# SinOncology/BreakID

Hardware: AMD Instinct MI355X
Metric: M reads/s clustered+split-scanned (higher is better)
Workload: dtype int32/u8 (+f64 sd replay)

## Files before the change

### breakid_amd/capi.py

```python
from __future__ import annotations

import ctypes as C
import math
import os
import subprocess

import numpy as np

from . import abi

_HERE = os.path.dirname(os.path.abspath(__file__))
LIB_PATH = os.path.join(_HERE, "libbreakid_hip.so")
_LIB = None


class BreakIDError(RuntimeError):
    def __init__(self, code, msg):
        super().__init__("libbreakid_hip error %d: %s" % (code, msg))
        self.code = code


def build(verbose=False):
    cmd = ["make", "-C", os.path.join(_HERE, "csrc"), "-j8"]
    r = subprocess.run(cmd, capture_output=not verbose, text=True)
    if r.returncode != 0:
        raise RuntimeError("building libbreakid_hip.so failed:\n" + (r.stdout or "")[-4000:] + (r.stderr or "")[-4000:])


EXPORTS = ["bk_init", "bk_prepare_process", "bk_free", "bk_last_error", "bk_set_stream", "bk_sync", "bk_get_stream", "bk_upload_records", "bk_records", "bk_exclude_regions", "bk_isize_stats",
           "bk_discordant_pairs", "bk_mask_and_cluster", "bk_split_evidence", "bk_cluster_summary",
           "bk_split_breakpoints", "bk_normal_support", "bk_ref_support", "bk_genotype_call", "bk_clip_support", "bk_clip_reads", "bk_base_depth", "bk_clip_rescue", "bk_junctions", "bk_junction_sides", "bk_vcf_breakend_alt", "bk_evidence", "bk_unique_support", "bk_clip_consensus", "bk_junction_fit", "bk_locus_similarity", "bk_site_complexity", "bk_window_coverage", "bk_window_context", "bk_call_windows", "bk_fusion_frame", "bk_link_calls", "bk_locus_partners", "bk_call_partner_sites", "bk_fragment_sizes", "bk_fragment_bounds", "bk_known_calls", "bk_split_junctions", "bk_split_junction_counts", "bk_debug_split_junctions", "bk_cigar_gaps", "bk_cigar_gap_counts", "bk_run", "bk_fetch", "bk_timing", "bk_timing_enable", "bk_timing_touched", "bk_group_stats", "bk_qname_hash", "bk_qname_check",
           "bk_bam_open", "bk_bam_header", "bk_bam_decode", "bk_bam_close", "bk_bam_extract", "bk_bam_names_free", "bk_bam_reads", "bk_reads_free", "bk_bam_decode_device", "bk_bam_decode_device_part", "bk_bam_decode_device_ctx", "bk_bam_dev_free", "bk_feed_release_caches", "bk_debug_bgzf_inflate", "bk_debug_std_sort", "bk_debug_scan", "bk_debug_radix_sort", "bk_debug_prims_info", "bk_sort_forms", "bk_debug_ahc", "bk_debug_points", "bk_debug_points_groups", "bk_debug_cluster_info", "bk_debug_stream_info", "bk_debug_stream_blocks", "bk_debug_cigar", "bk_debug_vote", "bk_debug_region", "bk_shard_begin", "bk_shard_get_stats", "bk_shard_set_stats",
           "bk_shard_sd_local", "bk_shard_sd_finish", "bk_shard_buffer", "bk_shard_set_buffer", "bk_shard_group_sizes",
           "bk_shard_own_groups", "bk_shard_route_candidates", "bk_shard_group_keys", "bk_shard_route_pairs", "bk_shard_group_pairs", "bk_shard_bp_cov", "bk_shard_bp_vote", "bk_shard_bp_vote_slice", "bk_shard_bp_set_voted", "bk_shard_bp_depth", "bk_shard_bp_finish"]


def lib():
    global _LIB
    if _LIB is None:
        if not os.path.exists(LIB_PATH):
            raise BreakIDError(abi.BK_ERR_NO_DEVICE, "libbreakid_hip.so is not built (run __graft_entry__.build()); "
                                                     "there is no CPU fallback")
        try:
            import torch
        except Exception:
            pass
        L = C.CDLL(LIB_PATH)
        vp, u64p, dp = C.c_void_p, C.POINTER(C.c_uint64), C.POINTER(C.c_double)
        L.bk_init.argtypes = [C.c_int, vp, C.POINTER(C.c_char_p), C.c_int, C.POINTER(vp)]
        L.bk_free.argtypes = [vp]
        L.bk_last_error.restype = C.c_char_p
        L.bk_last_error.argtypes = [vp]
        L.bk_set_stream.argtypes = [vp, vp]
        L.bk_sync.argtypes = [vp]
        L.bk_upload_records.argtypes = [vp, C.POINTER(abi.Soa), C.c_int]
# ... 26 lines not shown
        L.bk_window_context.argtypes = [vp, vp, C.c_uint64, C.c_int, C.POINTER(vp)]
        L.bk_call_windows.argtypes = [vp, C.c_int, C.c_int, C.c_uint32, vp, vp]
        L.bk_fusion_frame.argtypes = [vp, C.POINTER(abi.TxModel), vp, C.c_uint64, C.POINTER(vp)]
        L.bk_link_calls.argtypes = [vp, vp, C.c_uint64, C.c_uint32, C.POINTER(vp)]
        L.bk_locus_partners.argtypes = [vp, vp, C.c_uint64, C.c_uint32, C.POINTER(vp)]
        L.bk_call_partner_sites.argtypes = [vp, C.c_double, vp]
        L.bk_fragment_sizes.argtypes = [vp, vp, C.c_uint64, C.c_int32, C.c_int32, C.POINTER(vp)]
        L.bk_fragment_bounds.argtypes = [C.c_double, C.c_double, C.POINTER(C.c_int32), C.POINTER(C.c_int32)]
        L.bk_known_calls.argtypes = [vp, vp, C.c_uint64, vp, C.c_uint64, C.c_uint32, C.POINTER(vp)]
        L.bk_split_junctions.argtypes = [vp, C.c_int, C.c_uint32, C.c_uint32, C.POINTER(vp), u64p]
        L.bk_split_junction_counts.argtypes = [vp, u64p]
        L.bk_debug_split_junctions.argtypes = [vp, C.c_int, C.c_uint32, C.c_uint32, vp, C.c_uint64, C.POINTER(vp), u64p]
        L.bk_cigar_gaps.argtypes = [vp, C.c_int, C.c_uint32, C.c_uint32, C.c_uint32, C.c_uint32, C.POINTER(vp), u64p]
        L.bk_cigar_gap_counts.argtypes = [vp, u64p]
        L.bk_fetch.argtypes = [vp, C.c_int, C.POINTER(vp), u64p, C.POINTER(C.POINTER(C.c_uint64)), C.POINTER(C.c_uint32)]
        L.bk_timing.argtypes = [vp, C.POINTER(C.POINTER(C.c_char_p)), C.POINTER(C.POINTER(C.c_float)),
                                C.POINTER(C.POINTER(C.c_uint64)), C.POINTER(C.c_int)]
        L.bk_timing_enable.argtypes = [vp, C.c_int]
        L.bk_timing_touched.argtypes = [vp, C.POINTER(C.POINTER(C.c_uint64)), C.POINTER(C.c_int)]
        L.bk_debug_std_sort.argtypes = [vp, vp, vp, C.c_uint32, vp]
        L.bk_debug_scan.argtypes = [vp, C.c_int, vp, C.c_uint64, C.c_int, vp]
        L.bk_debug_radix_sort.argtypes = [vp, vp, vp, C.c_uint64, C.c_int, C.c_int, vp, vp]
        L.bk_debug_prims_info.argtypes = [u64p]
        L.bk_sort_forms.argtypes = [vp, u64p]
        L.bk_debug_ahc.argtypes = [vp, vp, vp, C.c_uint32, C.c_double, vp, vp, C.POINTER(C.c_uint32)]
        L.bk_debug_points.argtypes = [vp, C.c_int, vp, vp, C.c_uint32, C.c_double, vp, vp, C.POINTER(C.c_uint32)]
        L.bk_debug_points_groups.argtypes = [vp, C.c_int, vp, vp, vp, C.c_uint32, C.c_double, vp, vp, vp, C.POINTER(C.c_uint32)]
        L.bk_debug_cluster_info.argtypes = [u64p]
        L.bk_debug_stream_info.argtypes = [u64p]
        L.bk_debug_stream_blocks.argtypes = [C.c_uint]
        L.bk_debug_cigar.argtypes = [vp, C.c_uint32, vp, vp, vp, vp, vp, vp, vp]
        L.bk_debug_vote.argtypes = [vp, vp, C.c_uint32, vp, C.c_uint32, C.c_int32, C.c_int32, vp]
        L.bk_debug_region.argtypes = [vp, C.c_int32, C.c_uint32, C.c_uint32, C.c_uint64, vp, C.c_uint32, C.POINTER(C.c_uint32), C.POINTER(C.c_uint32),
                                      C.POINTER(C.c_uint32)]
        L.bk_shard_begin.argtypes = [vp, C.c_uint64, C.c_int]
        L.bk_shard_get_stats.argtypes = [vp, C.POINTER(abi.ShardStats)]
        L.bk_shard_set_stats.argtypes = [vp, C.POINTER(abi.ShardStats)]
        L.bk_shard_sd_local.argtypes = [vp, u64p, C.POINTER(vp), u64p]
        L.bk_shard_sd_finish.argtypes = [vp, vp, C.c_uint64, C.c_uint64, dp, dp]
        L.bk_shard_buffer.argtypes = [vp, C.c_int, C.POINTER(vp), u64p, C.POINTER(C.c_uint32)]
        L.bk_shard_set_buffer.argtypes = [vp, C.c_int, vp, C.c_uint64]
        L.bk_shard_group_sizes.argtypes = [vp, C.POINTER(C.POINTER(C.c_uint64)), C.POINTER(C.c_uint32)]
        L.bk_shard_own_groups.argtypes = [vp, vp, C.c_uint32]
        L.bk_shard_route_candidates.argtypes = [vp, C.c_uint32, C.POINTER(vp), C.POINTER(C.POINTER(C.c_uint64))]
        L.bk_shard_group_keys.argtypes = [vp, C.POINTER(C.POINTER(C.c_uint32)), C.POINTER(C.c_uint32)]
        L.bk_shard_route_pairs.argtypes = [vp, vp, C.c_uint32, C.c_uint32, C.POINTER(vp), C.POINTER(C.POINTER(C.c_uint64))]
# ... 71 lines not shown
    rc = M.bk_multi_run(C.byref(soa), lens.ctypes.data, names, len(contigs), int(n_gpus), int(transport), int(qual), int(fast), C.byref(w), C.byref(ncl), C.byref(h), err, 512)
    if rc != 0:
        raise BreakIDError(rc, err.value.decode())
    try:
        mean, sd = C.c_double(), C.c_double()
        rc = M.bk_multi_stats(h, C.byref(mean), C.byref(sd), None, None)
        if rc != 0:
            raise BreakIDError(rc, "bk_multi_stats")
        L = lib()
        clusters, _ = abi.fetch_array(L, h, lambda hh, st, d, c, g, ng: L.bk_fetch(hh, st, d, c, g, ng), abi.STAGE_CLUSTERS)
        return {"w": w.value, "n_clustered": ncl.value, "mean": mean.value, "sd": sd.value, "clusters": clusters}
    finally:
        M.bk_multi_free(h)


def prims_info():
    out = (C.c_uint64 * 4)()
    rc = lib().bk_debug_prims_info(out)
    if rc != 0:
        raise BreakIDError(rc, "bk_debug_prims_info")
    return dict(zip(("BLOCK", "SCAN_TILE", "SCAN_ONE_MAX", "RS_TILE"), (int(v) for v in out)))


def cluster_info():
    out = (C.c_uint64 * 2)()
    rc = lib().bk_debug_cluster_info(out)
    if rc != 0:
        raise BreakIDError(rc, "bk_debug_cluster_info")
    return dict(zip(("FW_TILE", "FW_LEVELS"), (int(v) for v in out)))


def stream_info():
    out = (C.c_uint64 * 4)()
    rc = lib().bk_debug_stream_info(out)
    if rc != 0:
        raise BreakIDError(rc, "bk_debug_stream_info")
    return dict(zip(("STREAM_V", "ST_CAND_CAP", "ST_SA_CAP", "RESIDENT"), (int(v) for v in out)))


def stream_blocks(blocks):
    rc = lib().bk_debug_stream_blocks(int(blocks))
    if rc != 0:
        raise BreakIDError(rc, "bk_debug_stream_blocks")


def w_from(mean, sd):
# ... 471 lines not shown

    def debug_std_sort(self, key, group_off):
        key = np.ascontiguousarray(key, np.uint32)
        group_off = np.ascontiguousarray(group_off, np.uint64)
        perm = np.zeros(len(key), np.uint32)
        self._check(self.L.bk_debug_std_sort(self.h, key.ctypes.data, group_off.ctypes.data, len(group_off) - 1, perm.ctypes.data))
        return perm

    def debug_scan(self, values, in_place=False):
        values = np.ascontiguousarray(values)
        assert values.ndim == 1 and values.dtype in (np.uint32, np.uint64), values.dtype
        out = np.zeros(len(values) + 1, values.dtype)
        self._check(self.L.bk_debug_scan(self.h, values.dtype.itemsize, values.ctypes.data if len(values) else None, len(values), int(in_place), out.ctypes.data))
        return out

    def debug_radix_sort(self, keys, vals, begin_bit, end_bit):
        keys = np.ascontiguousarray(keys, np.uint64)
        vals = np.ascontiguousarray(vals, np.uint32)
        assert keys.ndim == 1 and keys.shape == vals.shape
        n = len(keys)
        ko, vo = np.zeros(n, np.uint64), np.zeros(n, np.uint32)
        self._check(self.L.bk_debug_radix_sort(self.h, keys.ctypes.data if n else None, vals.ctypes.data if n else None, n, int(begin_bit), int(end_bit),
                                               ko.ctypes.data if n else None, vo.ctypes.data if n else None))
        return ko, vo

    def sort_forms(self):
        out = (C.c_uint64 * 3)()
        self._check(self.L.bk_sort_forms(self.h, out))
        return tuple(int(v) for v in out)

    def debug_ahc(self, x, y, w):
        x = np.ascontiguousarray(x, np.uint32)
        y = np.ascontiguousarray(y, np.uint32)
        n = len(x)
        idx = np.zeros(max(n, 1), np.uint32)
        cl = np.zeros(max(n, 1), np.int32)
        m = C.c_uint32()
        self._check(self.L.bk_debug_ahc(self.h, x.ctypes.data, y.ctypes.data, n, float(w), idx.ctypes.data, cl.ctypes.data, C.byref(m)))
        return idx[:m.value].copy(), cl[:m.value].copy()

    def debug_points(self, mode, x, y, w):
        x = np.ascontiguousarray(x, np.uint32)
        y = np.ascontiguousarray(y, np.uint32)
        n = len(x)
        idx = np.zeros(max(n, 1), np.uint32)
        cl = np.zeros(max(n, 1), np.int32)
# ... 308 lines not shown
```

### breakid_amd/csrc/api.hip

```cpp
#include <algorithm>
#include <cmath>
#include <limits>
#include <cstring>
#include <numeric>

#include "bk_common.h"
#include "prims.h"
#include "stream.h"
#include "join.h"
#include "cluster.h"
#include "bp.h"
#include "normal.h"
#include "genotype.h"
#include "clip.h"
#include "junction.h"
#include "evidence.h"
#include "unique.h"
#include "consensus.h"
#include "jfit.h"
#include "locsim.h"
#include "seqcx.h"
#include "coverage.h"
#include "context.h"
#include "frame.h"
// ... 130 lines not shown
  std::vector<struct bk_window_cov> f_wincov;
  CtxBufs cxb;
  std::vector<struct bk_window_ctx> f_winctx;
  FrameBufs frb;
  std::vector<struct bk_frame_call> f_frame;
  LinkBufs lkb;
  std::vector<struct bk_call_link> f_link;
  PartnerBufs ptb;
  std::vector<struct bk_locus_partners> f_partners;
  FragBufs fgb;
  std::vector<struct bk_frag_sizes> f_fragsize;
  KnownBufs knb;
  std::vector<struct bk_known_call> f_known;
  SjBufs sjb;
  SjStats sj_stats;
  std::vector<SjClaim> sj_claims;
  bool sj_claims_valid = false;
  std::vector<struct bk_split_junction> f_sj;
  GapBufs gpb;
  GapStats gap_stats;
  std::vector<struct bk_cigar_gap> f_gaps;

  prims::RadixBufs dbg_radix;
  DevBuf dbg_in, dbg_out, dbg_vals;

  std::vector<bk_pair> f_pairs[3];
  std::vector<uint64_t> f_off[3];
  std::vector<bk_split> f_splits;
  std::vector<bk_cluster> f_clusters;
  std::vector<int32_t> f_gkeys;
  std::vector<bk_group_stat> f_gstats;

  bool timing = false;
  std::vector<StageTimer> timers;
  Timing tout;

  void tick(const char *name, uint64_t bytes, bool begin, uint64_t touched = 0)
  {
    if (!timing) return;
    if (begin)
    {
      StageTimer t;
      t.name = name;
      t.bytes = bytes;
      t.touched = touched;
      HIP_CHECK(hipEventCreate(&t.a));
// ... 2203 lines not shown
    prims::RadixBufs &rb = ctx->dbg_radix;
    uint64_t *dk = ctx->dbg_in.as<uint64_t>(n);
    uint32_t *dv = ctx->dbg_vals.as<uint32_t>(n);
    HIP_CHECK(hipMemsetAsync(rb.keys_alt.as<uint64_t>(n), 0xA5, n * 8, ctx->st));
    HIP_CHECK(hipMemsetAsync(rb.vals_alt.as<uint32_t>(n), 0xA5, n * 4, ctx->st));
    HIP_CHECK(hipMemcpyAsync(dk, keys, n * 8, hipMemcpyHostToDevice, ctx->st));
    HIP_CHECK(hipMemcpyAsync(dv, vals, n * 4, hipMemcpyHostToDevice, ctx->st));
    uint64_t *ko = nullptr;
    uint32_t *vo = nullptr;
    prims::radix_sort_pairs(dk, dv, n, begin_bit, end_bit, rb, ctx->st, &ko, &vo);
    HIP_CHECK(hipMemcpyAsync(keys_out, ko, n * 8, hipMemcpyDeviceToHost, ctx->st));
    HIP_CHECK(hipMemcpyAsync(vals_out, vo, n * 4, hipMemcpyDeviceToHost, ctx->st));
    HIP_CHECK(hipStreamSynchronize(ctx->st));
  });
}

int bk_debug_prims_info(uint64_t out[4])
{
  if (!out) return BK_ERR_ARG;
  out[0] = prims::BLOCK;
  out[1] = prims::SCAN_TILE;
  out[2] = prims::SCAN_ONE_MAX;
  out[3] = prims::RS_TILE;
  return BK_OK;
}

int bk_sort_forms(bk_ctx *ctx, uint64_t out[3])
{
  return guarded(ctx, [&] {
    if (!out) throw bk_error(BK_ERR_ARG, "bk_sort_forms: null output");
    ctx->stage.sort_forms(out);
  });
}

int bk_debug_ahc(bk_ctx *ctx, const uint32_t *x, const uint32_t *y, uint32_t n, double w, uint32_t *idx_out, int32_t *cluster_out, uint32_t *n_out)
{
  return guarded(ctx, [&] {
    if (!x || !y || !idx_out || !cluster_out || !n_out) throw bk_error(BK_ERR_ARG, "bk_debug_ahc: null argument");
    std::vector<bk_pair> hp(n);
    for (uint32_t i = 0; i < n; ++i)
    {
      memset(&hp[i], 0, sizeof(bk_pair));
      hp[i].x = x[i];
      hp[i].y = y[i];
    }
    DevBuf dp, dcl;
// ... 436 lines not shown
```

### breakid_amd/csrc/bp.h

```cpp
#pragma once
#include "bk_common.h"
#include "prims.h"

template <class Less> __device__ __forceinline__ uint64_t wave_lower(uint64_t lo, uint64_t hi, Less less)
{
  const uint32_t lane = threadIdx.x & 63;
  while (hi - lo > 64)
  {
    const uint64_t width = hi - lo;
    const uint64_t p = lo + width * (lane + 1) / 65;
    const uint32_t c = (uint32_t) __popcll(__ballot(less(p)));
    const uint64_t nlo = c ? lo + width * c / 65 + 1 : lo;
    const uint64_t nhi = c < 64 ? lo + width * (c + 1) / 65 : hi;
    lo = nlo;
    hi = nhi;
  }
  const uint64_t i = lo + lane;
  return lo + (uint64_t) __popcll(__ballot(i < hi && less(i)));
}
__device__ __forceinline__ uint32_t wave_sum_u32(uint32_t v)
{
  for (int d = 32; d; d >>= 1) v += (uint32_t) __shfl_xor((int) v, d, 64);
  return v;
}

// ... 26 lines not shown
  {
    const unsigned long long want = rec_key(T, P < -0x80000000ll ? -0x80000000ll : P);
    const unsigned long long *__restrict__ samp = r.samp;
    const uint64_t a = wave_lower(0, r.n_samp, [&](uint64_t m) { return samp[m] < want; });
    lo = a ? ((a - 1) << REC_SAMPLE_SHIFT) + 1 : 0;
    hi = a < r.n_samp ? (a << REC_SAMPLE_SHIFT) : r.n;
  }
  const uint32_t Tu = (uint32_t) T;
  return wave_lower(lo, hi, [&](uint64_t m) {
    const uint32_t t = (uint32_t) r.tid[m];
    return t != Tu ? (t < Tu) : ((long long) r.pos[m] < P);
  });
}

struct BpWork
{
  uint64_t t1lo, t1hi, t2lo, t2hi;
  uint32_t ok, pad;
};

struct BpBufs
{
  DevBuf samp, key, val, kmax, lexbase, slotbase, an, as1, as2, amin1, amax1, amin2, amax2, atype, keep, off, tmpc, work, nmatch, moff, err, emit, ecount, scan_tmp, cov, depth, voted, nvalid, maxrec;
  prims::RadixBufs radix;
};

uint64_t count_valid_clusters(const bk_cluster *cl, uint64_t ncl, BpBufs &b, hipStream_t st);
void sort_splits(bk_split *unsorted, uint64_t n, bk_split *sorted, BpBufs &b, hipStream_t st, int rec_bits);
uint64_t cluster_summary(const bk_pair *pairs, const uint32_t *idx, const uint32_t *gof, const uint32_t *cl, uint64_t n, uint32_t ng, const uint32_t *gkey,
                         const uint32_t *glex, const uint32_t *lex_to_num, int32_t nt, double w, DevBuf &clusters_out, BpBufs &b, hipStream_t st);
RecView rec_sampled(const RecView &r, DevBuf &samp, hipStream_t st);
uint32_t *bp_cov_partial(const RecView &r, const bk_cluster *cl, uint64_t ncl, double w, int maxspan, BpBufs &b, hipStream_t st);
void bp_vote(const bk_split *sp, uint64_t nsp, bk_cluster *cl, uint64_t ncl, double w, int maxspan, const uint32_t *cov, const int32_t *hdr_id, BpBufs &b, hipStream_t st);
uint32_t *bp_depth_partial(const RecView &r, const bk_cluster *cl, uint64_t ncl, int maxspan, BpBufs &b, hipStream_t st);
void base_depth_at(const RecView &r, const int32_t *tid, const uint32_t *pos, uint64_t n, int maxspan, DevBuf &samp, hipStream_t st, uint32_t *depth);
void bp_finish(bk_cluster *cl, uint64_t ncl, const uint32_t *depth, BpBufs &b, hipStream_t st);
void split_breakpoints(const RecView &r, const bk_split *sp, uint64_t nsp, bk_cluster *cl, uint64_t ncl, double w, int maxspan, const int32_t *hdr_id, BpBufs &b,
                       hipStream_t st);
void debug_region(const RecView &r, const bk_split *sp, uint64_t nsp, int32_t tid, uint32_t start, uint32_t end, int maxspan, unsigned long long depth_pos, bk_split *out,
                  uint32_t cap, uint32_t *res, hipStream_t st);
```

### breakid_amd/csrc/bp.hip

```cpp
#include "bk_common.h"
#include "prims.h"
#include "bp.h"
#include <algorithm>
#include <vector>

namespace
{
__global__ __launch_bounds__(256) void k_group_kmax(const uint32_t *__restrict__ gof, const uint32_t *__restrict__ cl, uint64_t n, uint32_t *__restrict__ kmax)
{
  uint64_t p = (uint64_t) blockIdx.x * blockDim.x + threadIdx.x;
  const bool live = p < n;
  uint32_t g = live ? gof[p] : 0xFFFFFFFFu;
  uint32_t v = live ? cl[p] + 1 : 0u;
  __shared__ uint32_t s_g[4], s_v[4];
  const uint32_t g0 = __shfl(g, 0, 64);
  const bool wave_uniform = __ballot(live && g != g0) == 0ull;
  if (wave_uniform)
    for (int d = 32; d; d >>= 1) v = max(v, (uint32_t) __shfl_xor((int) v, d, 64));
  if ((threadIdx.x & 63) == 0)
  {
    s_g[threadIdx.x >> 6] = wave_uniform ? g0 : 0xFFFFFFFEu;
    s_v[threadIdx.x >> 6] = v;
  }
  __syncthreads();
// ... 586 lines not shown

void sort_splits(bk_split *unsorted, uint64_t n, bk_split *sorted, BpBufs &b, hipStream_t st, int rec_bits)
{
  if (n == 0) return;
  uint64_t *key = b.key.as<uint64_t>(n);
  uint32_t *val = b.val.as<uint32_t>(n);
  unsigned long long *mx = nullptr;
  if (rec_bits <= 0)
  {
    mx = b.maxrec.as<unsigned long long>(2);
    HIP_CHECK(hipMemsetAsync(mx, 0, 8, st));
  }
  hipLaunchKernelGGL(k_split_keys, dim3(nb(n)), dim3(256), 0, st, unsorted, n, key, val, mx);
  if (mx)
  {
    unsigned long long h = 0;
    HIP_CHECK(hipMemcpyAsync(&h, mx, 8, hipMemcpyDeviceToHost, st));
    HIP_CHECK(hipStreamSynchronize(st));
    rec_bits = 1;
    while (rec_bits < 64 && (h >> rec_bits) != 0ull) ++rec_bits;
  }
  uint64_t *ks;
  uint32_t *vs;
  prims::radix_sort_pairs(key, val, n, 0, rec_bits, b.radix, st, &ks, &vs);
  hipLaunchKernelGGL(k_split_gather, dim3(nb(n)), dim3(256), 0, st, unsorted, vs, n, sorted);
}

uint64_t cluster_summary(const bk_pair *pairs, const uint32_t *idx, const uint32_t *gof, const uint32_t *cl, uint64_t n, uint32_t ng, const uint32_t *gkey,
                         const uint32_t *glex, const uint32_t *lex_to_num, int32_t nt, double w, DevBuf &clusters_out, BpBufs &b, hipStream_t st)
{
  if (n == 0 || ng == 0) return 0;
  uint32_t *kmax = b.kmax.as<uint32_t>((uint64_t) ng + 1);
  HIP_CHECK(hipMemsetAsync(kmax, 0, ((uint64_t) ng + 1) * 4, st));
  hipLaunchKernelGGL(k_group_kmax, dim3(nb(n)), dim3(256), 0, st, gof, cl, n, kmax);
  uint32_t *slotbase = b.slotbase.as<uint32_t>((uint64_t) ng + 1), *lexbase = b.lexbase.as<uint32_t>((uint64_t) ng + 1);
  hipLaunchKernelGGL(k_slot_bases, dim3(1), dim3(prims::BLOCK), 0, st, kmax, lex_to_num, ng, lexbase, slotbase);
  uint32_t nslots = 0;
  HIP_CHECK(hipMemcpyAsync(&nslots, lexbase + ng, 4, hipMemcpyDeviceToHost, st));
  HIP_CHECK(hipStreamSynchronize(st));
  if (nslots == 0) return 0;
  ClusterAcc acc;
  acc.n = b.an.as<uint32_t>(nslots);
  acc.sum1 = b.as1.as<unsigned long long>(nslots);
  acc.sum2 = b.as2.as<unsigned long long>(nslots);
  acc.min1 = b.amin1.as<uint32_t>(nslots);
  acc.max1 = b.amax1.as<uint32_t>(nslots);
  acc.min2 = b.amin2.as<uint32_t>(nslots);
// ... 147 lines not shown
```

### breakid_amd/csrc/join.h

```cpp
#pragma once
#include "bk_common.h"
#include "prims.h"
#include <vector>

struct JoinBufs
{
  DevBuf counter, unsorted, okey, oval, key, val, pairs, gof, gflag, gscan, gstart, gkey, scan_tmp, route_cand, route_cnt, route_pairs, route_off, maxrec, key2, val2;
  prims::RadixBufs radix;
  int rec_bits = 32;
  int rec_bits_eff = 32;
};

struct JoinResult
{
  uint64_t n_pairs = 0;
  uint32_t n_groups = 0;
  bk_pair *pairs = nullptr;
  uint32_t *gof = nullptr;
  uint64_t *gstart = nullptr;
  uint32_t *gkey = nullptr;
};

void join_candidates(const Cand *cand, uint64_t n_cand, double w, const uint32_t *tprefix, int32_t nt, JoinBufs &b, hipStream_t st, JoinResult &res);
void join_assign_ids(JoinResult &res, const uint32_t *glex_dev, hipStream_t st);

Cand *route_candidates(const Cand *cand, uint64_t n, uint32_t world, JoinBufs &b, hipStream_t st, std::vector<uint64_t> &counts);
bk_pair *route_pairs(const JoinResult &jr, const std::vector<uint64_t> &off_of_group, JoinBufs &b, hipStream_t st);
void group_pairs(const bk_pair *raw, uint64_t np, int32_t nt, JoinBufs &b, hipStream_t st, JoinResult &res);
```

### breakid_amd/csrc/join.hip

```cpp
#include "bk_common.h"
#include "prims.h"
#include "join.h"

namespace
{
__global__ __launch_bounds__(256) void k_join_keys(const Cand *__restrict__ c, uint64_t n, uint64_t *__restrict__ key, uint32_t *__restrict__ val)
{
  uint64_t i = (uint64_t) blockIdx.x * blockDim.x + threadIdx.x;
  if (i < n)
  {
    key[i] = c[i].qhash;
    val[i] = (uint32_t) i;
  }
}

__global__ __launch_bounds__(256) void k_join_rec_keys(const Cand *__restrict__ c, uint64_t n, uint64_t *__restrict__ key, uint32_t *__restrict__ val)
{
  uint64_t i = (uint64_t) blockIdx.x * blockDim.x + threadIdx.x;
  if (i < n)
  {
    key[i] = c[i].rec;
    val[i] = (uint32_t) i;
  }
}
// ... 310 lines not shown
{
  if (n_cand > 0xFFFFFFF0ull) throw bk_error(BK_ERR_LIMIT, "more than 2^32 discordant candidates");
  const int rec_bits = effective_rec_bits(cand, n_cand, k_max_rec_cand, nt, b, st);
  unsigned long long *counter = b.counter.as<unsigned long long>(2);
  uint32_t *err = (uint32_t *) (counter + 1);
  HIP_CHECK(hipMemsetAsync(counter, 0, 16, st));
  uint64_t cap = n_cand / 2 + 1;
  bk_pair *unsorted = b.unsorted.as<bk_pair>(cap);
  uint64_t *okey = b.okey.as<uint64_t>(cap);
  uint32_t *oval = b.oval.as<uint32_t>(cap);
  unsigned long long host[2] = {0, 0};
  static const int first_attempt = getenv("BK_JOIN_ATTEMPT") ? std::max(0, std::min(2, atoi(getenv("BK_JOIN_ATTEMPT")))) : 0;
  for (int attempt = first_attempt; attempt < 3; ++attempt)
  {
    if (n_cand)
    {
      uint64_t *key = b.key.as<uint64_t>(n_cand);
      uint32_t *val = b.val.as<uint32_t>(n_cand);
      uint64_t *ks;
      uint32_t *vs;
      if (attempt < 2)
      {
        hipLaunchKernelGGL(k_join_keys, dim3(cdiv(n_cand, 256)), dim3(256), 0, st, cand, n_cand, key, val);
        prims::radix_sort_pairs(key, val, n_cand, attempt == 0 ? 32 : 0, 64, b.radix, st, &ks, &vs);
        if (attempt == 0) hipLaunchKernelGGL(k_join_fix_runs, dim3(cdiv(n_cand, 256)), dim3(256), 0, st, ks, vs, n_cand, err);
      }
      else
      {
        hipLaunchKernelGGL(k_join_rec_keys, dim3(cdiv(n_cand, 256)), dim3(256), 0, st, cand, n_cand, key, val);
        prims::radix_sort_pairs(key, val, n_cand, 0, rec_bits, b.radix, st, &ks, &vs);
        uint64_t *key2 = b.key2.as<uint64_t>(n_cand);
        uint32_t *val2 = b.val2.as<uint32_t>(n_cand);
        hipLaunchKernelGGL(k_join_hash_of, dim3(cdiv(n_cand, 256)), dim3(256), 0, st, cand, (const uint32_t *) vs, n_cand, key2, val2);
        prims::radix_sort_pairs(key2, val2, n_cand, 0, 64, b.radix, st, &ks, &vs);
      }
      hipLaunchKernelGGL(k_join_pairs, dim3(cdiv(n_cand, 256)), dim3(256), 0, st, cand, ks, vs, n_cand, w, tprefix, nt, unsorted, okey, oval,
                         (unsigned long long) cap, counter, err, rec_bits, attempt == 2 ? 1 : 0);
    }
    HIP_CHECK(hipMemcpyAsync(host, counter, 16, hipMemcpyDeviceToHost, st));
    HIP_CHECK(hipStreamSynchronize(st));
    if (attempt == 0 && ((uint32_t) host[1] & 4u))
    {
      HIP_CHECK(hipMemsetAsync(counter, 0, 16, st));
      continue;
    }
    if (attempt < 2 && ((uint32_t) host[1] & 1u) && !((uint32_t) host[1] & 2u))
    {
      HIP_CHECK(hipMemsetAsync(counter, 0, 16, st));
      attempt = 1;
      continue;
    }
    break;
  }
  if ((uint32_t) host[1] & 2u)
    throw bk_error(BK_ERR_COLLISION, "two different read names share one 64-bit name hash (their second hashes differ): the mate join would not be the reference's");
  if ((uint32_t) host[1] & 1u) throw bk_error(BK_ERR_HIP, "mate join: a run was refused although its candidates were sorted (internal error)");
  if (host[0] > cap) throw bk_error(BK_ERR_LIMIT, "pair capacity exceeded");
  return host[0];
}

static void group_sorted(const bk_pair *unsorted, uint64_t *okey, uint32_t *oval, uint64_t np, int32_t nt, JoinBufs &b, hipStream_t st, JoinResult &res)
{
  res = JoinResult();
  res.n_pairs = np;
  bk_pair *pairs = b.pairs.as<bk_pair>(np + 1);
  uint32_t *gof = b.gof.as<uint32_t>(np + 1);
  res.pairs = pairs;
  res.gof = gof;
  if (np == 0) return;
  int gbits = 1;
  while ((1ull << gbits) < (uint64_t) (nt + 1) * (uint64_t) (nt + 1) && gbits < 32) ++gbits;
  uint64_t *ks;
  uint32_t *vs;
  const int rbits = b.rec_bits_eff;
  prims::radix_sort_pairs(okey, oval, np, 0, rbits + gbits, b.radix, st, &ks, &vs);
  uint32_t *gflag = b.gflag.as<uint32_t>(np + 1);
  uint32_t *gscan = b.gscan.as<uint32_t>(np + 1);
  hipLaunchKernelGGL(k_gather_pairs, dim3(cdiv(np, 256)), dim3(256), 0, st, unsorted, vs, ks, np, pairs, gflag, rbits);
  prims::exclusive_scan<uint32_t>(gflag, gscan, np, b.scan_tmp, st);
  uint32_t ng = 0;
  HIP_CHECK(hipMemcpyAsync(&ng, gscan + np, 4, hipMemcpyDeviceToHost, st));
  HIP_CHECK(hipStreamSynchronize(st));
  res.n_groups = ng;
  uint64_t *gstart = b.gstart.as<uint64_t>((uint64_t) ng + 1);
  uint32_t *gkey = b.gkey.as<uint32_t>((uint64_t) ng + 1);
  hipLaunchKernelGGL(k_group_starts, dim3(cdiv(np, 256)), dim3(256), 0, st, gflag, gscan, ks, np, gstart, gkey, gof, rbits);
  res.gstart = gstart;
  res.gkey = gkey;
}

void join_candidates(const Cand *cand, uint64_t n_cand, double w, const uint32_t *tprefix, int32_t nt, JoinBufs &b, hipStream_t st, JoinResult &res)
{
  const uint64_t np = join_raw_pairs(cand, n_cand, w, tprefix, nt, b, st);
  group_sorted(b.unsorted.get<bk_pair>(), b.okey.get<uint64_t>(), b.oval.get<uint32_t>(), np, nt, b, st, res);
}

void group_pairs(const bk_pair *raw, uint64_t np, int32_t nt, JoinBufs &b, hipStream_t st, JoinResult &res)
{
// ... 52 lines not shown
```

### include/breakid_hip.h

```cpp
#ifndef BREAKID_HIP_H
#define BREAKID_HIP_H

#include <stdint.h>
#include <stddef.h>

#ifdef __cplusplus
extern "C" {
#endif

#define BK_OK 0
#define BK_ERR_ARG (-1)
#define BK_ERR_HIP (-2)
#define BK_ERR_NO_DEVICE (-3)
#define BK_ERR_UNSORTED (-4)
#define BK_ERR_CIGAR (-5)
#define BK_ERR_IO (-6)
#define BK_ERR_LIMIT (-7)
#define BK_ERR_COLLISION (-8)

#define BK_MEM_HOST 0
#define BK_MEM_DEVICE 1

typedef struct bk_ctx bk_ctx;

// ... 314 lines not shown
int bk_shard_sd_local(bk_ctx *ctx, uint64_t *l_total, void **ex_dev, uint64_t *n_ex);
int bk_shard_sd_finish(bk_ctx *ctx, const void *all_ex_dev, uint64_t n_all, uint64_t l_grand, double *mean, double *sd);
int bk_shard_buffer(bk_ctx *ctx, int which, void **dev, uint64_t *count, uint32_t *elem_bytes);
int bk_shard_set_buffer(bk_ctx *ctx, int which, const void *dev, uint64_t count);
int bk_shard_group_sizes(bk_ctx *ctx, const uint64_t **starts, uint32_t *n_groups);
int bk_shard_own_groups(bk_ctx *ctx, const uint8_t *own, uint32_t n_groups);
int bk_shard_route_candidates(bk_ctx *ctx, uint32_t world, void **dev, const uint64_t **counts);
int bk_shard_group_keys(bk_ctx *ctx, const uint32_t **keys, uint32_t *n_groups);
int bk_shard_route_pairs(bk_ctx *ctx, const uint32_t *dest_of_group, uint32_t n_groups, uint32_t world, void **dev, const uint64_t **counts);
int bk_shard_group_pairs(bk_ctx *ctx, const void *pairs_dev, uint64_t n, const uint32_t *all_keys, uint32_t n_all_keys);
int bk_shard_bp_cov(bk_ctx *ctx, double w, void **cov_dev, uint64_t *n);
int bk_shard_bp_vote(bk_ctx *ctx, double w, const void *cov_total_dev);
int bk_shard_bp_vote_slice(bk_ctx *ctx, double w, const void *cov_total_dev, uint64_t lo, uint64_t hi, void **clusters_dev, void **voted_dev);
int bk_shard_bp_set_voted(bk_ctx *ctx, const void *voted_all_dev);
int bk_shard_bp_depth(bk_ctx *ctx, void **depth_dev, uint64_t *n);
int bk_shard_bp_finish(bk_ctx *ctx, const void *depth_total_dev);

int bk_debug_std_sort(bk_ctx *ctx, const uint32_t *key, const uint64_t *group_off, uint32_t n_groups, uint32_t *perm_out);

int bk_debug_scan(bk_ctx *ctx, int elem_bytes, const void *in, uint64_t n, int in_place, void *out);
int bk_debug_radix_sort(bk_ctx *ctx, const uint64_t *keys, const uint32_t *vals, uint64_t n, int begin_bit, int end_bit, uint64_t *keys_out, uint32_t *vals_out);
int bk_debug_prims_info(uint64_t out[4]);

int bk_sort_forms(bk_ctx *ctx, uint64_t out[3]);

int bk_debug_ahc(bk_ctx *ctx, const uint32_t *x, const uint32_t *y, uint32_t n, double w, uint32_t *idx_out, int32_t *cluster_out, uint32_t *n_out);

int bk_debug_points(bk_ctx *ctx, int mode, const uint32_t *x, const uint32_t *y, uint32_t n, double w, uint32_t *idx_out, int32_t *cluster_out, uint32_t *n_out);
int bk_debug_points_groups(bk_ctx *ctx, int mode, const uint32_t *x, const uint32_t *y, const uint64_t *group_off, uint32_t n_groups, double w, uint32_t *idx_out,
                           int32_t *cluster_out, uint64_t *goff_out, uint32_t *n_out);
int bk_debug_cluster_info(uint64_t out[2]);
int bk_debug_stream_info(uint64_t out[4]);
int bk_debug_stream_blocks(unsigned blocks);
int bk_debug_cigar(bk_ctx *ctx, uint32_t n, const uint8_t *kind, const uint32_t *c1_off, const uint8_t *c1, const uint32_t *c2_off, const uint8_t *c2, const int32_t *e,
                   int32_t *out6);
int bk_debug_vote(bk_ctx *ctx, const bk_split *side1, uint32_t n1, const bk_split *side2, uint32_t n2, int32_t p1_tid, int32_t p2_tid, int32_t *out3);
int bk_debug_region(bk_ctx *ctx, int32_t tid, uint32_t start, uint32_t end, uint64_t depth_pos, bk_split *out, uint32_t cap, uint32_t *n_out, uint32_t *cov_out,
                    uint32_t *depth_out);

typedef struct bk_bam bk_bam;
uint64_t bk_qname_hash(const char *name, size_t len);
uint32_t bk_qname_check(const char *name, size_t len);
int bk_bam_open(const char *path, bk_bam **out, char *err, size_t errlen);
int bk_bam_header(const bk_bam *b, int *n_targets, const char *const **names, const uint32_t **lens);
int bk_bam_decode(bk_bam *b, bk_soa *out, char *err, size_t errlen);
void bk_bam_close(bk_bam *b);
// ... 24 lines not shown
```

Measured before the change: 11660.

## Replace join and split radix sorts with wide-tile 8-bit-digit onesweep-style sorter

Adds a new LSD radix sort for 64-bit keys with 32-bit values. Each block handles a large tile (512 threads × 16 rows), builds a histogram with wave-uniform atomics, and scatters through shared memory after ranking digits with ballots, using evenly balanced 8-bit digit widths per pass. The join candidate sorts, the pair grouping sort and the split-evidence sort all switch from the old radix sort to this path. The aim is fewer passes and launches and more coalesced global writes, at the cost of heavy register and LDS use per block, which may lower occupancy.

```diff
diff --git a/breakid_amd/capi.py b/breakid_amd/capi.py
--- a/breakid_amd/capi.py
+++ b/breakid_amd/capi.py
@@ -30,7 +30,7 @@
 EXPORTS = ["bk_init", "bk_prepare_process", "bk_free", "bk_last_error", "bk_set_stream", "bk_sync", "bk_get_stream", "bk_upload_records", "bk_records", "bk_exclude_regions", "bk_isize_stats",
            "bk_discordant_pairs", "bk_mask_and_cluster", "bk_split_evidence", "bk_cluster_summary",
            "bk_split_breakpoints", "bk_normal_support", "bk_ref_support", "bk_genotype_call", "bk_clip_support", "bk_clip_reads", "bk_base_depth", "bk_clip_rescue", "bk_junctions", "bk_junction_sides", "bk_vcf_breakend_alt", "bk_evidence", "bk_unique_support", "bk_clip_consensus", "bk_junction_fit", "bk_locus_similarity", "bk_site_complexity", "bk_window_coverage", "bk_window_context", "bk_call_windows", "bk_fusion_frame", "bk_link_calls", "bk_locus_partners", "bk_call_partner_sites", "bk_fragment_sizes", "bk_fragment_bounds", "bk_known_calls", "bk_split_junctions", "bk_split_junction_counts", "bk_debug_split_junctions", "bk_cigar_gaps", "bk_cigar_gap_counts", "bk_run", "bk_fetch", "bk_timing", "bk_timing_enable", "bk_timing_touched", "bk_group_stats", "bk_qname_hash", "bk_qname_check",
-           "bk_bam_open", "bk_bam_header", "bk_bam_decode", "bk_bam_close", "bk_bam_extract", "bk_bam_names_free", "bk_bam_reads", "bk_reads_free", "bk_bam_decode_device", "bk_bam_decode_device_part", "bk_bam_decode_device_ctx", "bk_bam_dev_free", "bk_feed_release_caches", "bk_debug_bgzf_inflate", "bk_debug_std_sort", "bk_debug_scan", "bk_debug_radix_sort", "bk_debug_prims_info", "bk_sort_forms", "bk_debug_ahc", "bk_debug_points", "bk_debug_points_groups", "bk_debug_cluster_info", "bk_debug_stream_info", "bk_debug_stream_blocks", "bk_debug_cigar", "bk_debug_vote", "bk_debug_region", "bk_shard_begin", "bk_shard_get_stats", "bk_shard_set_stats",
+           "bk_bam_open", "bk_bam_header", "bk_bam_decode", "bk_bam_close", "bk_bam_extract", "bk_bam_names_free", "bk_bam_reads", "bk_reads_free", "bk_bam_decode_device", "bk_bam_decode_device_part", "bk_bam_decode_device_ctx", "bk_bam_dev_free", "bk_feed_release_caches", "bk_debug_bgzf_inflate", "bk_debug_std_sort", "bk_debug_scan", "bk_debug_radix_sort", "bk_debug_prims_info", "bk_debug_radix_sort_wide", "bk_debug_prims_wide_info", "bk_sort_forms", "bk_debug_ahc", "bk_debug_points", "bk_debug_points_groups", "bk_debug_cluster_info", "bk_debug_stream_info", "bk_debug_stream_blocks", "bk_debug_cigar", "bk_debug_vote", "bk_debug_region", "bk_shard_begin", "bk_shard_get_stats", "bk_shard_set_stats",
            "bk_shard_sd_local", "bk_shard_sd_finish", "bk_shard_buffer", "bk_shard_set_buffer", "bk_shard_group_sizes",
            "bk_shard_own_groups", "bk_shard_route_candidates", "bk_shard_group_keys", "bk_shard_route_pairs", "bk_shard_group_pairs", "bk_shard_bp_cov", "bk_shard_bp_vote", "bk_shard_bp_vote_slice", "bk_shard_bp_set_voted", "bk_shard_bp_depth", "bk_shard_bp_finish"]
 
@@ -103,6 +103,8 @@
         L.bk_debug_scan.argtypes = [vp, C.c_int, vp, C.c_uint64, C.c_int, vp]
         L.bk_debug_radix_sort.argtypes = [vp, vp, vp, C.c_uint64, C.c_int, C.c_int, vp, vp]
         L.bk_debug_prims_info.argtypes = [u64p]
+        L.bk_debug_radix_sort_wide.argtypes = [vp, vp, vp, C.c_uint64, C.c_int, C.c_int, vp, vp]
+        L.bk_debug_prims_wide_info.argtypes = [u64p]
         L.bk_sort_forms.argtypes = [vp, u64p]
         L.bk_debug_ahc.argtypes = [vp, vp, vp, C.c_uint32, C.c_double, vp, vp, C.POINTER(C.c_uint32)]
         L.bk_debug_points.argtypes = [vp, C.c_int, vp, vp, C.c_uint32, C.c_double, vp, vp, C.POINTER(C.c_uint32)]
@@ -220,6 +222,14 @@
     return dict(zip(("BLOCK", "SCAN_TILE", "SCAN_ONE_MAX", "RS_TILE"), (int(v) for v in out)))
 
 
+def prims_wide_info():
+    out = (C.c_uint64 * 4)()
+    rc = lib().bk_debug_prims_wide_info(out)
+    if rc != 0:
+        raise BreakIDError(rc, "bk_debug_prims_wide_info")
+    return dict(zip(("WIDE_TILE", "WIDE_BLOCK", "WIDE_DIGIT_BITS", "WIDE_ONE_SCAN_KEYS"), (int(v) for v in out)))
+
+
 def cluster_info():
     out = (C.c_uint64 * 2)()
     rc = lib().bk_debug_cluster_info(out)
@@ -737,6 +747,16 @@
         ko, vo = np.zeros(n, np.uint64), np.zeros(n, np.uint32)
         self._check(self.L.bk_debug_radix_sort(self.h, keys.ctypes.data if n else None, vals.ctypes.data if n else None, n, int(begin_bit), int(end_bit),
                                                ko.ctypes.data if n else None, vo.ctypes.data if n else None))
+        return ko, vo
+
+    def debug_radix_sort_wide(self, keys, vals, begin_bit, end_bit):
+        keys = np.ascontiguousarray(keys, np.uint64)
+        vals = np.ascontiguousarray(vals, np.uint32)
+        assert keys.ndim == 1 and keys.shape == vals.shape
+        n = len(keys)
+        ko, vo = np.zeros(n, np.uint64), np.zeros(n, np.uint32)
+        self._check(self.L.bk_debug_radix_sort_wide(self.h, keys.ctypes.data if n else None, vals.ctypes.data if n else None, n, int(begin_bit), int(end_bit),
+                                                    ko.ctypes.data if n else None, vo.ctypes.data if n else None))
         return ko, vo
 
     def sort_forms(self):
diff --git a/breakid_amd/csrc/api.hip b/breakid_amd/csrc/api.hip
--- a/breakid_amd/csrc/api.hip
+++ b/breakid_amd/csrc/api.hip
@@ -176,6 +176,7 @@
   std::vector<struct bk_cigar_gap> f_gaps;
 
   prims::RadixBufs dbg_radix;
+  prims::WideRadixBufs dbg_wide;
   DevBuf dbg_in, dbg_out, dbg_vals;
 
   std::vector<bk_pair> f_pairs[3];
@@ -2425,6 +2426,39 @@
   out[1] = prims::SCAN_TILE;
   out[2] = prims::SCAN_ONE_MAX;
   out[3] = prims::RS_TILE;
+  return BK_OK;
+}
+
+int bk_debug_radix_sort_wide(bk_ctx *ctx, const uint64_t *keys, const uint32_t *vals, uint64_t n, int begin_bit, int end_bit, uint64_t *keys_out, uint32_t *vals_out)
+{
+  return guarded(ctx, [&] {
+    if (n && (!keys || !vals || !keys_out || !vals_out)) throw bk_error(BK_ERR_ARG, "bk_debug_radix_sort_wide: null argument");
+    if (begin_bit < 0 || end_bit > 64) throw bk_error(BK_ERR_ARG, "bk_debug_radix_sort_wide: bits outside [0, 64]");
+    prims::radix_check_count(n);
+    if (!n) return;
+    prims::WideRadixBufs &rb = ctx->dbg_wide;
+    uint64_t *dk = ctx->dbg_in.as<uint64_t>(n);
+    uint32_t *dv = ctx->dbg_vals.as<uint32_t>(n);
+    HIP_CHECK(hipMemsetAsync(rb.keys_alt.as<uint64_t>(n), 0xA5, n * 8, ctx->st));
+    HIP_CHECK(hipMemsetAsync(rb.vals_alt.as<uint32_t>(n), 0xA5, n * 4, ctx->st));
+    HIP_CHECK(hipMemcpyAsync(dk, keys, n * 8, hipMemcpyHostToDevice, ctx->st));
+    HIP_CHECK(hipMemcpyAsync(dv, vals, n * 4, hipMemcpyHostToDevice, ctx->st));
+    uint64_t *ko = nullptr;
+    uint32_t *vo = nullptr;
+    prims::radix_sort_pairs_wide(dk, dv, n, begin_bit, end_bit, rb, ctx->st, &ko, &vo);
+    HIP_CHECK(hipMemcpyAsync(keys_out, ko, n * 8, hipMemcpyDeviceToHost, ctx->st));
+    HIP_CHECK(hipMemcpyAsync(vals_out, vo, n * 4, hipMemcpyDeviceToHost, ctx->st));
+    HIP_CHECK(hipStreamSynchronize(ctx->st));
+  });
+}
+
+int bk_debug_prims_wide_info(uint64_t out[4])
+{
+  if (!out) return BK_ERR_ARG;
+  out[0] = prims::WIDE_TILE;
+  out[1] = prims::WIDE_BLOCK;
+  out[2] = prims::WIDE_DIGIT_BITS;
+  out[3] = (uint64_t) prims::WIDE_TILE * (prims::SCAN_ONE_MAX >> prims::WIDE_DIGIT_BITS);
   return BK_OK;
 }
 
diff --git a/breakid_amd/csrc/bp.h b/breakid_amd/csrc/bp.h
--- a/breakid_amd/csrc/bp.h
+++ b/breakid_amd/csrc/bp.h
@@ -1,6 +1,7 @@
 #pragma once
 #include "bk_common.h"
 #include "prims.h"
+#include "prims_wide.h"
 
 template <class Less> __device__ __forceinline__ uint64_t wave_lower(uint64_t lo, uint64_t hi, Less less)
 {
@@ -73,7 +74,7 @@
 struct BpBufs
 {
   DevBuf samp, key, val, kmax, lexbase, slotbase, an, as1, as2, amin1, amax1, amin2, amax2, atype, keep, off, tmpc, work, nmatch, moff, err, emit, ecount, scan_tmp, cov, depth, voted, nvalid, maxrec;
-  prims::RadixBufs radix;
+  prims::WideRadixBufs wide;
 };
 
 uint64_t count_valid_clusters(const bk_cluster *cl, uint64_t ncl, BpBufs &b, hipStream_t st);
diff --git a/breakid_amd/csrc/bp.hip b/breakid_amd/csrc/bp.hip
--- a/breakid_amd/csrc/bp.hip
+++ b/breakid_amd/csrc/bp.hip
@@ -632,7 +632,7 @@
   }
   uint64_t *ks;
   uint32_t *vs;
-  prims::radix_sort_pairs(key, val, n, 0, rec_bits, b.radix, st, &ks, &vs);
+  prims::radix_sort_pairs_wide(key, val, n, 0, rec_bits, b.wide, st, &ks, &vs);
   hipLaunchKernelGGL(k_split_gather, dim3(nb(n)), dim3(256), 0, st, unsorted, vs, n, sorted);
 }
 
diff --git a/breakid_amd/csrc/join.h b/breakid_amd/csrc/join.h
--- a/breakid_amd/csrc/join.h
+++ b/breakid_amd/csrc/join.h
@@ -1,12 +1,14 @@
 #pragma once
 #include "bk_common.h"
 #include "prims.h"
+#include "prims_wide.h"
 #include <vector>
 
 struct JoinBufs
 {
   DevBuf counter, unsorted, okey, oval, key, val, pairs, gof, gflag, gscan, gstart, gkey, scan_tmp, route_cand, route_cnt, route_pairs, route_off, maxrec, key2, val2;
   prims::RadixBufs radix;
+  prims::WideRadixBufs wide;
   int rec_bits = 32;
   int rec_bits_eff = 32;
 };
diff --git a/breakid_amd/csrc/join.hip b/breakid_amd/csrc/join.hip
--- a/breakid_amd/csrc/join.hip
+++ b/breakid_amd/csrc/join.hip
@@ -356,17 +356,17 @@
       if (attempt < 2)
       {
         hipLaunchKernelGGL(k_join_keys, dim3(cdiv(n_cand, 256)), dim3(256), 0, st, cand, n_cand, key, val);
-        prims::radix_sort_pairs(key, val, n_cand, attempt == 0 ? 32 : 0, 64, b.radix, st, &ks, &vs);
+        prims::radix_sort_pairs_wide(key, val, n_cand, attempt == 0 ? 32 : 0, 64, b.wide, st, &ks, &vs);
         if (attempt == 0) hipLaunchKernelGGL(k_join_fix_runs, dim3(cdiv(n_cand, 256)), dim3(256), 0, st, ks, vs, n_cand, err);
       }
       else
       {
         hipLaunchKernelGGL(k_join_rec_keys, dim3(cdiv(n_cand, 256)), dim3(256), 0, st, cand, n_cand, key, val);
-        prims::radix_sort_pairs(key, val, n_cand, 0, rec_bits, b.radix, st, &ks, &vs);
+        prims::radix_sort_pairs_wide(key, val, n_cand, 0, rec_bits, b.wide, st, &ks, &vs);
         uint64_t *key2 = b.key2.as<uint64_t>(n_cand);
         uint32_t *val2 = b.val2.as<uint32_t>(n_cand);
         hipLaunchKernelGGL(k_join_hash_of, dim3(cdiv(n_cand, 256)), dim3(256), 0, st, cand, (const uint32_t *) vs, n_cand, key2, val2);
-        prims::radix_sort_pairs(key2, val2, n_cand, 0, 64, b.radix, st, &ks, &vs);
+        prims::radix_sort_pairs_wide(key2, val2, n_cand, 0, 64, b.wide, st, &ks, &vs);
       }
       hipLaunchKernelGGL(k_join_pairs, dim3(cdiv(n_cand, 256)), dim3(256), 0, st, cand, ks, vs, n_cand, w, tprefix, nt, unsorted, okey, oval,
                          (unsigned long long) cap, counter, err, rec_bits, attempt == 2 ? 1 : 0);
@@ -407,7 +407,7 @@
   uint64_t *ks;
   uint32_t *vs;
   const int rbits = b.rec_bits_eff;
-  prims::radix_sort_pairs(okey, oval, np, 0, rbits + gbits, b.radix, st, &ks, &vs);
+  prims::radix_sort_pairs_wide(okey, oval, np, 0, rbits + gbits, b.wide, st, &ks, &vs);
   uint32_t *gflag = b.gflag.as<uint32_t>(np + 1);
   uint32_t *gscan = b.gscan.as<uint32_t>(np + 1);
   hipLaunchKernelGGL(k_gather_pairs, dim3(cdiv(np, 256)), dim3(256), 0, st, unsorted, vs, ks, np, pairs, gflag, rbits);
diff --git a/breakid_amd/csrc/prims_wide.h b/breakid_amd/csrc/prims_wide.h
--- /dev/null
+++ b/breakid_amd/csrc/prims_wide.h
@@ -0,0 +1,221 @@
+#pragma once
+#include "prims.h"
+
+namespace prims
+{
+constexpr int WIDE_BLOCK = 512;
+constexpr int WIDE_WAVES = WIDE_BLOCK / BK_WAVE;
+constexpr int WIDE_ROWS = 16;
+constexpr int WIDE_TILE = WIDE_BLOCK * WIDE_ROWS;
+constexpr int WIDE_DIGIT_BITS = 8;
+constexpr int WIDE_BINS = 1 << WIDE_DIGIT_BITS;
+static_assert(WIDE_BINS <= WIDE_BLOCK, "a thread per bin");
+
+__device__ __forceinline__ void wide_hist_add(uint32_t *hist, uint32_t d, bool valid)
+{
+  if (!valid) d = 0xFFFFFFFFu;
+  const uint32_t d0 = __builtin_amdgcn_readfirstlane(d);
+  if (__all(d == d0))
+  {
+    if (valid && (threadIdx.x & 63) == 0) atomicAdd(&hist[d0], 64u);
+  }
+  else if (valid)
+    atomicAdd(&hist[d], 1u);
+}
+
+static __global__ __launch_bounds__(WIDE_BLOCK) void k_wide_hist(const uint64_t *__restrict__ keys, uint32_t *__restrict__ ghist, uint64_t n, int shift, uint32_t mask,
+                                                                 uint32_t nb)
+{
+  __shared__ uint32_t hist[WIDE_BINS];
+  if (threadIdx.x <= mask) hist[threadIdx.x] = 0;
+  __syncthreads();
+  const uint64_t base = (uint64_t) blockIdx.x * WIDE_TILE;
+  if (base + WIDE_TILE <= n && ((uintptr_t) keys & 15) == 0)
+  {
+    const ulonglong2 *k2 = (const ulonglong2 *) (keys + base);
+#pragma unroll
+    for (int k = 0; k < WIDE_ROWS / 2; ++k)
+    {
+      const ulonglong2 v = k2[k * WIDE_BLOCK + threadIdx.x];
+      wide_hist_add(hist, (uint32_t) (v.x >> shift) & mask, true);
+      wide_hist_add(hist, (uint32_t) (v.y >> shift) & mask, true);
+    }
+  }
+  else
+  {
+#pragma unroll
+    for (int k = 0; k < WIDE_ROWS; ++k)
+    {
+      const uint64_t i = base + (uint64_t) k * WIDE_BLOCK + threadIdx.x;
+      const bool valid = i < n;
+      wide_hist_add(hist, valid ? ((uint32_t) (keys[i] >> shift) & mask) : 0u, valid);
+    }
+  }
+  __syncthreads();
+  if (threadIdx.x <= mask) ghist[(uint64_t) threadIdx.x * nb + blockIdx.x] = hist[threadIdx.x];
+}
+
+static __global__ __launch_bounds__(WIDE_BLOCK, WIDE_BLOCK / 128) void k_wide_scatter(const uint64_t *__restrict__ kin, const uint32_t *__restrict__ vin, uint64_t *__restrict__ kout,
+                                                                                       uint32_t *__restrict__ vout, const uint32_t *__restrict__ goff, uint64_t n, int shift,
+                                                                                       uint32_t mask, uint32_t nb)
+{
+  constexpr int D = WIDE_BINS;
+  constexpr int STAGE_WORDS = WIDE_TILE * 2 > WIDE_WAVES * D ? WIDE_TILE * 2 : WIDE_WAVES * D;
+  __shared__ __attribute__((aligned(16))) uint32_t stage[STAGE_WORDS];
+  __shared__ uint32_t gdelta[D];
+  __shared__ uint32_t wsum[WIDE_WAVES];
+  uint32_t *whist = stage;
+  uint64_t *skeys = (uint64_t *) stage;
+  uint32_t *svals = stage;
+  const int w = threadIdx.x >> 6, lane = threadIdx.x & 63;
+  if (threadIdx.x <= mask)
+#pragma unroll
+    for (int i = 0; i < WIDE_WAVES; ++i) whist[i * D + threadIdx.x] = 0;
+  __syncthreads();
+  const uint64_t tile0 = (uint64_t) blockIdx.x * WIDE_TILE;
+  const uint32_t cnt = n - tile0 < (uint64_t) WIDE_TILE ? (uint32_t) (n - tile0) : (uint32_t) WIDE_TILE;
+  const uint32_t row0 = (uint32_t) w * WIDE_ROWS * 64 + lane;
+  uint64_t key[WIDE_ROWS];
+  uint32_t val[WIDE_ROWS], pos[WIDE_ROWS];
+  const uint64_t lt = (1ull << lane) - 1ull;
+#pragma unroll
+  for (int r = 0; r < WIDE_ROWS; ++r)
+  {
+    const uint32_t t = row0 + (uint32_t) r * 64;
+    const bool valid = t < cnt;
+    key[r] = valid ? kin[tile0 + t] : 0ull;
+    val[r] = valid ? vin[tile0 + t] : 0u;
+  }
+#pragma unroll
+  for (int r = 0; r < WIDE_ROWS; ++r)
+  {
+    const bool valid = row0 + (uint32_t) r * 64 < cnt;
+    const uint32_t d = (uint32_t) (key[r] >> shift) & mask;
+    uint64_t peers = __ballot(valid);
+#pragma unroll
+    for (int b = 0; b < WIDE_DIGIT_BITS; ++b)
+    {
+      const bool bit = (d >> b) & 1u;
+      const uint64_t m = __ballot(bit);
+      peers &= bit ? m : ~m;
+    }
+    const uint32_t rk = __popcll(peers & lt);
+    const uint32_t c = __popcll(peers);
+    const int leader = valid ? (__ffsll((long long) peers) - 1) : lane;
+    uint32_t old = 0;
+    if (valid && lane == leader) old = atomicAdd(&whist[w * D + d], c);
+    old = __shfl(old, leader, 64);
+    pos[r] = old + rk;
+  }
+  __syncthreads();
+  {
+    const uint32_t d = threadIdx.x;
+    uint32_t tot = 0;
+    if (d <= mask)
+#pragma unroll
+      for (int i = 0; i < WIDE_WAVES; ++i) tot += whist[i * D + d];
+    const uint32_t inc = wave_inclusive_scan(tot);
+    if (lane == 63) wsum[w] = inc;
+    __syncthreads();
+    uint32_t at = inc - tot;
+#pragma unroll
+    for (int i = 0; i < WIDE_WAVES; ++i)
+      if (i < w) at += wsum[i];
+    if (d <= mask)
+    {
+      gdelta[d] = goff[(uint64_t) d * nb + blockIdx.x] - at;
+#pragma unroll
+      for (int i = 0; i < WIDE_WAVES; ++i)
+      {
+        const uint32_t c = whist[i * D + d];
+        whist[i * D + d] = at;
+        at += c;
+      }
+    }
+  }
+  __syncthreads();
+#pragma unroll
+  for (int r = 0; r < WIDE_ROWS; ++r)
+  {
+    const uint32_t d = (uint32_t) (key[r] >> shift) & mask;
+    if (row0 + (uint32_t) r * 64 < cnt) pos[r] += whist[w * D + d];
+  }
+  __syncthreads();
+#pragma unroll
+  for (int r = 0; r < WIDE_ROWS; ++r)
+    if (row0 + (uint32_t) r * 64 < cnt) skeys[pos[r]] = key[r];
+  __syncthreads();
+  uint32_t dst[WIDE_ROWS];
+#pragma unroll
+  for (int m = 0; m < WIDE_ROWS; ++m)
+  {
+    const uint32_t j = (uint32_t) m * WIDE_BLOCK + threadIdx.x;
+    dst[m] = 0;
+    if (j < cnt)
+    {
+      const uint64_t k = skeys[j];
+      dst[m] = gdelta[(uint32_t) (k >> shift) & mask] + j;
+      kout[dst[m]] = k;
+    }
+  }
+  __syncthreads();
+#pragma unroll
+  for (int r = 0; r < WIDE_ROWS; ++r)
+    if (row0 + (uint32_t) r * 64 < cnt) svals[pos[r]] = val[r];
+  __syncthreads();
+#pragma unroll
+  for (int m = 0; m < WIDE_ROWS; ++m)
+  {
+    const uint32_t j = (uint32_t) m * WIDE_BLOCK + threadIdx.x;
+    if (j < cnt) vout[dst[m]] = svals[j];
+  }
+}
+
+struct WideRadixBufs
+{
+  DevBuf keys_alt, vals_alt, hist, scan_tmp;
+};
+
+inline int wide_pass_widths(int bits, int widths[64])
+{
+  if (bits <= 0) return 0;
+  const int passes = (bits + WIDE_DIGIT_BITS - 1) / WIDE_DIGIT_BITS;
+  for (int p = 0; p < passes; ++p) widths[p] = bits / passes + (p < bits % passes ? 1 : 0);
+  return passes;
+}
+
+inline void wide_pass(const uint64_t *ka, const uint32_t *va, uint64_t *kb, uint32_t *vb, uint32_t *hist, uint64_t n, int shift, int width, uint32_t nb,
+                                         DevBuf &scan_tmp, hipStream_t st)
+{
+  const uint32_t mask = (1u << width) - 1u;
+  hipLaunchKernelGGL(k_wide_hist, dim3(nb), dim3(WIDE_BLOCK), 0, st, ka, hist, n, shift, mask, nb);
+  exclusive_scan<uint32_t>(hist, hist, ((uint64_t) mask + 1) * nb, scan_tmp, st);
+  hipLaunchKernelGGL(k_wide_scatter, dim3(nb), dim3(WIDE_BLOCK), 0, st, ka, va, kb, vb, hist, n, shift, mask, nb);
+}
+
+inline void radix_sort_pairs_wide(uint64_t *keys, uint32_t *vals, uint64_t n, int begin_bit, int end_bit, WideRadixBufs &rb, hipStream_t st, uint64_t **keys_out,
+                                  uint32_t **vals_out)
+{
+  *keys_out = keys;
+  *vals_out = vals;
+  if (n == 0 || end_bit <= begin_bit) return;
+  radix_check_count(n);
+  int widths[64];
+  const int passes = wide_pass_widths(end_bit - begin_bit, widths);
+  uint64_t *ka = keys, *kb = rb.keys_alt.as<uint64_t>(n);
+  uint32_t *va = vals, *vb = rb.vals_alt.as<uint32_t>(n);
+  const uint32_t nb = cdiv(n, WIDE_TILE);
+  uint32_t *hist = rb.hist.as<uint32_t>(((uint64_t) 1 << widths[0]) * nb + 1);
+  int shift = begin_bit;
+  for (int p = 0; p < passes; ++p)
+  {
+    wide_pass(ka, va, kb, vb, hist, n, shift, widths[p], nb, rb.scan_tmp, st);
+    shift += widths[p];
+    std::swap(ka, kb);
+    std::swap(va, vb);
+  }
+  *keys_out = ka;
+  *vals_out = va;
+}
+
+}
diff --git a/include/breakid_hip.h b/include/breakid_hip.h
--- a/include/breakid_hip.h
+++ b/include/breakid_hip.h
@@ -360,6 +360,9 @@
 int bk_debug_radix_sort(bk_ctx *ctx, const uint64_t *keys, const uint32_t *vals, uint64_t n, int begin_bit, int end_bit, uint64_t *keys_out, uint32_t *vals_out);
 int bk_debug_prims_info(uint64_t out[4]);
 
+int bk_debug_radix_sort_wide(bk_ctx *ctx, const uint64_t *keys, const uint32_t *vals, uint64_t n, int begin_bit, int end_bit, uint64_t *keys_out, uint32_t *vals_out);
+int bk_debug_prims_wide_info(uint64_t out[4]);
+
 int bk_sort_forms(bk_ctx *ctx, uint64_t out[3]);
 
 int bk_debug_ahc(bk_ctx *ctx, const uint32_t *x, const uint32_t *y, uint32_t n, double w, uint32_t *idx_out, int32_t *cluster_out, uint32_t *n_out);
```

After: 11840 (median of 6 runs). 1.02x the previous value.
